# swyoon/Diffusion-by-MaxEntIRL

Hardware: AMD Instinct MI355X
Metric: images/sec (CIFAR-10 DDPM T=10 generation) (higher is better)
Workload: dtype bf16; 1 GPU; CIFAR-10 DDPM U-Net (35.7M params) VARSampler T=10 generation, 256 images/GPU/step, 3x32x32 (BASELINE configs[1]); noise drawn inside the step; global_batch=256, T=10, parallelism=dp1 (independent trajectories, no collective)

## Files before the change

diffusion-by-maxentirl_amd/dxmi_hip/_lib.py:

```python
import ctypes
import os

_HERE = os.path.dirname(os.path.abspath(__file__))
LIB_PATH = os.environ.get("DXMI_LIB") or os.path.join(_HERE, "libdxmi_hip.so")

c_void_p, c_int, c_float, c_int64 = ctypes.c_void_p, ctypes.c_int32, ctypes.c_float, ctypes.c_int64


class ConvDesc(ctypes.Structure):

    _fields_ = [
        ("in0", c_void_p), ("in1", c_void_p), ("wpacked", c_void_p), ("bias", c_void_p),
        ("addvec", c_void_p), ("residual", c_void_p), ("out", c_void_p),
        ("N", c_int), ("IH", c_int), ("IW", c_int), ("C0", c_int), ("C1", c_int),
        ("OH", c_int), ("OW", c_int), ("Cout", c_int),
        ("ksize", c_int), ("stride", c_int), ("pad", c_int), ("upsample", c_int), ("act", c_int),
        ("addvec_ld", c_int), ("in_mode", c_int), ("out_mode", c_int), ("variant", c_int),
        ("mask_src", c_void_p), ("mask_slope", c_float), ("gn_stats", c_void_p),
        ("gn_out", c_void_p), ("gn_gamma", c_void_p), ("gn_beta", c_void_p), ("gn_eps", c_float), ("gn_groups", c_int), ("gn_flags", c_int),
    ]


class PackItem(ctypes.Structure):

    _fields_ = [("w", c_void_p), ("dst", c_void_p), ("Cout", c_int), ("Cin", c_int), ("ksize", c_int), ("transpose_flip", c_int),
                ("k27", c_int)]


SIGNATURES = {
    "dxmi_last_error": (ctypes.c_char_p, []),
    "dxmi_version": (c_int, []),
    "dxmi_device_check": (c_int, []),
    "dxmi_set_tuning": (c_int, [ctypes.c_char_p, c_int]),
    "dxmi_get_tuning": (c_int, [ctypes.c_char_p, ctypes.POINTER(c_int)]),
    "dxmi_conv2d_fwd": (c_int, [ctypes.POINTER(ConvDesc), c_void_p]),
    "dxmi_conv2d_kernel_id": (c_int, [ctypes.POINTER(ConvDesc)]),
    "dxmi_conv2d_gn_stats_partials": (c_int, [ctypes.POINTER(ConvDesc)]),
    "dxmi_conv2d_gn_fuse_supported": (c_int, [ctypes.POINTER(ConvDesc)]),
    "dxmi_conv_ws_last_clock": (c_int, [ctypes.POINTER(ctypes.c_uint64)]),
    "dxmi_gn_block_stats_partials": (c_int, [c_int]),
    "dxmi_gn_block_stats": (c_int, [c_void_p, c_void_p, c_int, c_int, c_int, c_void_p]),
    "dxmi_gn_stats_fold": (c_int, [c_void_p, c_void_p, c_int, c_int, c_int, c_int, c_void_p]),
    "dxmi_groupnorm_apply": (c_int, [c_void_p, c_int, c_void_p, c_int, c_void_p, c_int, c_void_p, c_int, c_void_p, c_void_p, c_void_p, c_int,
                                     c_void_p, c_int, c_int, c_int, c_float, c_int, c_void_p]),
    "dxmi_groupnorm_apply_split": (c_int, [c_void_p, c_int, c_void_p, c_int, c_void_p, c_int, c_void_p, c_int, c_void_p, c_void_p, c_void_p, c_int,
                                           c_void_p, c_void_p, c_int, c_int, c_int, c_float, c_int, c_void_p]),
    "dxmi_groupnorm_silu_shortcut_supported": (c_int, [ctypes.POINTER(ConvDesc), c_int]),
    "dxmi_groupnorm_silu_shortcut": (c_int, [ctypes.POINTER(ConvDesc), c_void_p, c_int, c_void_p, c_int, c_void_p, c_void_p, c_int, c_float,
                                             c_int, c_void_p, c_void_p, c_void_p]),
    "dxmi_gn_blockstats_to_generic": (c_int, [c_void_p, c_int, c_int, c_void_p, c_int, c_int, c_void_p, c_int, c_int, c_int, c_void_p]),
    "dxmi_attention_fwd_lse_supported": (c_int, [c_int, c_int, c_int]),
    "dxmi_attention_fwd_lse": (c_int, [c_void_p, c_void_p, c_void_p, c_int, c_int, c_int, c_int, c_float, c_void_p]),
    "dxmi_attention_bwd_lse": (c_int, [c_void_p, c_void_p, c_void_p, c_void_p, c_void_p, c_void_p, c_int, c_int, c_int, c_int, c_float, c_void_p]),
    "dxmi_gn_ss_grads": (c_int, [c_void_p, c_void_p, c_int, c_void_p, c_void_p, c_void_p, c_void_p, c_void_p, c_int, c_int, c_void_p]),
    "dxmi_fid_stats_workspace_bytes": (c_int64, [c_int64, c_int]),
    "dxmi_fid_stats": (c_int, [c_void_p, c_int64, c_int, c_void_p, c_void_p, c_void_p, c_void_p]),
    "dxmi_knn_radii_workspace_bytes": (c_int64, [c_int64, c_int, c_int, c_int]),
    "dxmi_knn_radii": (c_int, [c_void_p, c_int64, c_int, c_int, c_int, c_void_p, c_void_p, c_void_p]),
    "dxmi_pr_membership_workspace_bytes": (c_int64, [c_int64, c_int64]),
    "dxmi_pr_membership": (c_int, [c_void_p, c_int64, c_void_p, c_void_p, c_int64, c_void_p, c_int, c_void_p, c_void_p, c_void_p, c_void_p]),
    "dxmi_inception_score_workspace_bytes": (c_int64, [c_int64, c_int, c_int]),
    "dxmi_inception_score": (c_int, [c_void_p, c_int64, c_int, c_void_p, c_int, c_int, c_void_p, c_void_p, c_void_p]),
    "dxmi_packed_conv_weight_bytes": (c_int64, [c_int, c_int, c_int, c_int]),
    "dxmi_pack_conv_weights": (c_int, [ctypes.POINTER(PackItem), c_int, c_void_p]),
    "dxmi_pack_conv_weight": (c_int, [c_void_p, c_void_p, c_int, c_int, c_int, c_int, c_int, c_void_p]),
    "dxmi_conv2d_wgrad_workspace_bytes": (c_int64, [c_int] * 6),
    "dxmi_conv2d_wgrad_plan": (c_int, [c_int] * 12 + [c_void_p]),
    "dxmi_conv2d_wgrad": (c_int, [c_void_p, c_int, c_void_p, c_int, c_void_p, c_void_p, c_void_p] + [c_int] * 11 + [c_void_p]),
    "dxmi_conv2d_wgrad_bias": (c_int, [c_void_p, c_int, c_void_p, c_int, c_void_p, c_void_p, c_void_p, c_void_p] + [c_int] * 11 + [c_void_p]),
    "dxmi_groupnorm_silu_bwd": (c_int, [c_void_p, c_int, c_void_p, c_int] + [c_void_p] * 9 + [c_int, c_int, c_int, c_float, c_int, c_void_p]),
    "dxmi_bgemm_bf16": (c_int, [c_void_p, c_void_p, c_void_p, c_int, c_int, c_int, c_int64, c_int64, c_int, c_int, c_int64, c_int64, c_int, c_int, c_int64, c_int64, c_int, c_int, c_float, c_int, c_int, c_void_p]),
    "dxmi_softmax_bwd": (c_int, [c_void_p, c_void_p, c_void_p, c_void_p, c_int64, c_int, c_void_p]),
    "dxmi_attention_bwd_supported": (c_int, [c_int, c_int, c_int]),
    "dxmi_attention_bwd_workspace_bytes": (c_int64, [c_int, c_int, c_int]),
    "dxmi_attention_bwd": (c_int, [c_void_p, c_void_p, c_void_p, c_void_p, c_void_p, c_int, c_int, c_int, c_int, c_float, c_void_p]),
    "dxmi_colsum_bf16": (c_int, [c_void_p, c_void_p, c_void_p, c_int64, c_int, c_int, c_void_p]),
    "dxmi_colsum_blocks_bf16": (c_int, [c_void_p, c_void_p, c_int64, c_int, c_int, c_void_p]),
    "dxmi_colsum_f32": (c_int, [c_void_p, c_void_p, c_int, c_int, c_int, c_void_p]),
    "dxmi_pool_act_bwd": (c_int, [c_void_p, c_void_p, c_void_p, c_int, c_int, c_int, c_int, c_int, c_float, c_void_p]),
    "dxmi_value_head_bwd": (c_int, [c_void_p, c_void_p, c_void_p, c_void_p, c_void_p, c_int, c_int, c_int, c_void_p]),
    "dxmi_groupnorm_silu_fwd": (c_int, [c_void_p, c_int, c_void_p, c_int, c_void_p, c_void_p, c_void_p,
                                        c_int, c_int, c_int, c_float, c_int, c_void_p]),
    "dxmi_attention_fwd": (c_int, [c_void_p, c_void_p, c_int, c_int, c_int, c_int, c_float, c_void_p]),
    "dxmi_attention_proj_supported": (c_int, [c_int, c_int, c_int]),
    "dxmi_pack_attn_proj_weight": (c_int, [c_void_p, c_void_p, c_void_p]),
    "dxmi_attention_proj_fwd": (c_int, [c_void_p, c_void_p, c_void_p, c_void_p, c_void_p, c_void_p, c_int, c_int, c_int, c_int, c_float, c_void_p]),
    "dxmi_attn_block_supported": (c_int, [c_int, c_int, c_int, c_int]),
    "dxmi_attn_block_packed_bytes": (c_int64, []),
    "dxmi_attn_block_pack": (c_int, [c_void_p] * 7 + [c_float, c_void_p, c_void_p]),
    "dxmi_attn_block_fwd": (c_int, [c_void_p, c_void_p, c_int, c_void_p, c_void_p, c_float, c_void_p, c_void_p, c_void_p, c_int, c_int, c_int, c_void_p]),
    "dxmi_timestep_embedding": (c_int, [c_void_p, c_void_p, c_int, c_int, c_int, c_float, c_void_p]),
    "dxmi_linear_fwd": (c_int, [c_void_p, c_void_p, c_void_p, c_void_p, c_int, c_int, c_int, c_int, c_int, c_void_p]),
    "dxmi_linear_splitk_slices": (c_int, [c_int, c_int, c_int]),
    "dxmi_linear_splitk": (c_int, [c_void_p, c_void_p, c_void_p, c_int, c_int, c_int, c_int, c_void_p]),
    "dxmi_var_step_fwd": (c_int, [c_void_p] * 10 + [c_int, c_int, c_int, c_void_p]),
    "dxmi_var_step_bwd": (c_int, [c_void_p] * 9 + [c_int, c_int, c_void_p]),
    "dxmi_edm_step_bwd": (c_int, [c_void_p] * 7 + [c_int, c_int, c_float, c_void_p]),
    "dxmi_var_gather_sched": (c_int, [c_void_p] * 9 + [c_int, c_int, c_void_p]),
    "dxmi_pool_act": (c_int, [c_void_p, c_void_p, c_int, c_int, c_int, c_int, c_int, c_int, c_void_p]),
    "dxmi_value_head": (c_int, [c_void_p, c_void_p, c_void_p, c_void_p, c_void_p, c_void_p, c_int, c_int, c_int, c_void_p]),
    "dxmi_groupnorm_silu_supported": (c_int, [c_int, c_int, c_int, c_int]),
    "dxmi_groupnorm_silu_bwd_supported": (c_int, [c_int, c_int, c_int, c_int]),
# ... 85 lines not shown
```

diffusion-by-maxentirl_amd/dxmi_hip/ops.py:

```python
import ctypes
import os

import torch

from . import _lib
from . import graph as _graph
from ._lib import ConvDesc, check, load

ACT_NONE, ACT_LEAKY02, ACT_RELU, ACT_SILU = 0, 1, 2, 3
IN_NHWC_BF16, IN_NCHW_F32_K27 = 0, 1
OUT_NHWC_BF16, OUT_NCHW_F32 = 0, 1


_RAW_STREAM = getattr(torch._C, "_cuda_getCurrentRawStream", None)
_GET_DEVICE = getattr(torch._C, "_cuda_getDevice", None)


def _stream():
    if _RAW_STREAM is not None and _GET_DEVICE is not None:
        return ctypes.c_void_p(_RAW_STREAM(_GET_DEVICE()))
    return ctypes.c_void_p(torch.cuda.current_stream().cuda_stream)


def _tree_fingerprint(module):
# ... 604 lines not shown
    while st.P > MAX_APPLY_PARTIALS:
        N, P, C2, _ = st.buf.shape
        PG = (P + group - 1) // group
        out = torch.empty((N, PG, C2, 2), dtype=torch.float32, device=st.buf.device)
        _prof("groupnorm", "fold", 0.0, 4.0 * (st.buf.numel() + out.numel()), lambda: check(
            load().dxmi_gn_stats_fold(_ptr(st.buf), _ptr(out), N, P, C2 * 2, group, _stream()), "dxmi_gn_stats_fold"))
        st = BlockStats(out, PG)
    return st


def block_stats(x):
    _need_cuda(x)
    N, H, W, C = x.shape
    assert x.dtype == torch.bfloat16 and x.is_contiguous()
    lib = load()
    P = int(lib.dxmi_gn_block_stats_partials(H * W))
    st = BlockStats(torch.empty((N, P, C // 2, 2), dtype=torch.float32, device=x.device), P)
    _prof("groupnorm", "block_stats", 0.0, 2.0 * x.numel(), lambda: check(
        lib.dxmi_gn_block_stats(_ptr(x), _ptr(st.buf), N, H * W, C, _stream()), "dxmi_gn_block_stats"))
    return fold_stats(st) if P > MAX_APPLY_PARTIALS else st


GN_APPLY_SPLIT = os.environ.get("DXMI_GN_APPLY_SPLIT", "0") == "1"


def groupnorm_apply(x, st, gamma, beta, *, in1=None, st1=None, groups=32, eps=1e-6, silu=True, out=None, scale_shift=None):
    _need_cuda(x, in1, gamma, beta, out, st.buf, st1.buf if st1 is not None else None, scale_shift)
    N, H, W, C0 = x.shape
    C1 = in1.shape[3] if in1 is not None else 0
    C = C0 + C1
    assert x.dtype == torch.bfloat16 and x.is_contiguous() and (in1 is None or (in1.is_contiguous() and st1 is not None))
    assert gamma.dtype == torch.float32 and beta.dtype == torch.float32 and gamma.numel() == C
    assert tuple(st.buf.shape) == (N, st.P, C0 // 2, 2) and (st1 is None or tuple(st1.buf.shape) == (N, st1.P, C1 // 2, 2))
    ss_ld = 0
    if scale_shift is not None:
        assert scale_shift.dtype == torch.float32 and scale_shift.stride(-1) == 1 and scale_shift.shape[1] == 2 * C
        ss_ld = scale_shift.stride(0)
    if out is None:
        out = torch.empty((N, H, W, C), dtype=torch.bfloat16, device=x.device)
    if GN_APPLY_SPLIT:
        ab = torch.empty((N, C, 2), dtype=torch.float32, device=x.device)
        _prof("groupnorm", "apply", 0.0, 4.0 * N * H * W * C, lambda: check(
            load().dxmi_groupnorm_apply_split(_ptr(x), C0, _ptr(st.buf), st.P, _ptr(in1), C1, _ptr(st1.buf) if st1 is not None else None,
                                              st1.P if st1 is not None else 0, _ptr(gamma), _ptr(beta), _ptr(scale_shift), ss_ld, _ptr(out),
                                              _ptr(ab), N, H * W, groups, float(eps), int(silu), _stream()), "dxmi_groupnorm_apply_split"))
        return out
    _prof("groupnorm", "apply", 0.0, 4.0 * N * H * W * C, lambda: check(
        load().dxmi_groupnorm_apply(_ptr(x), C0, _ptr(st.buf), st.P, _ptr(in1), C1, _ptr(st1.buf) if st1 is not None else None,
                                    st1.P if st1 is not None else 0, _ptr(gamma), _ptr(beta), _ptr(scale_shift), ss_ld, _ptr(out),
                                    N, H * W, groups, float(eps), int(silu), _stream()), "dxmi_groupnorm_apply"))
    return out


def groupnorm_silu(x, gamma, beta, *, in1=None, groups=32, eps=1e-6, silu=True, out=None, scale_shift=None, stats=None, saved=None):
    _need_cuda(x, in1, gamma, beta, out, scale_shift)
    N, H, W, C0 = x.shape
    C1 = in1.shape[3] if in1 is not None else 0
    if stats is not None and stats[0] is not None and (in1 is None or stats[1] is not None) \
            and ((C0 + C1) // groups) % 2 == 0 and C0 % 8 == 0 and C1 % 8 == 0:
        if saved is not None:
            saved.append(gn_blockstats_to_generic(stats[0], stats[1] if in1 is not None else None, N, H * W, C0, C1, groups))
        return groupnorm_apply(x, stats[0], gamma, beta, in1=in1, st1=stats[1] if in1 is not None else None, groups=groups,
                               eps=eps, silu=silu, out=out, scale_shift=scale_shift)
    if scale_shift is not None or not load().dxmi_groupnorm_silu_supported(C0, C1, H * W, groups):
        return groupnorm_generic(x, gamma, beta, in1=in1, groups=groups, eps=eps, silu=silu, out=out, scale_shift=scale_shift, saved=saved)
    assert x.dtype == torch.bfloat16 and x.is_contiguous()
    assert gamma.dtype == torch.float32 and beta.dtype == torch.float32 and gamma.numel() == C0 + C1
    if out is None:
        out = torch.empty((N, H, W, C0 + C1), dtype=torch.bfloat16, device=x.device)
    _prof("groupnorm", "resident", 0.0, 4.0 * N * H * W * (C0 + C1), lambda: check(
        load().dxmi_groupnorm_silu_fwd(_ptr(x), C0, _ptr(in1), C1, _ptr(gamma), _ptr(beta), _ptr(out), N, H * W,
                                       groups, float(eps), int(silu), _stream()), "dxmi_groupnorm_silu_fwd"))
    return out


def groupnorm_silu_shortcut(x, gamma, beta, pw, *, in1=None, bias=None, groups=32, eps=1e-6, silu=True, stats=None):
    _need_cuda(x, in1, gamma, beta, bias)
    if stats is None or stats[0] is None or (in1 is not None and stats[1] is None) or pw.k27 or pw.ksize != 1:
        return None
    N, H, W, C0 = x.shape
    C1 = in1.shape[3] if in1 is not None else 0
    C = C0 + C1
    if (C // groups) % 2 != 0 or C0 % 8 != 0 or C1 % 8 != 0:
        return None
    assert x.dtype == torch.bfloat16 and x.is_contiguous() and C == pw.Cin
    assert in1 is None or (in1.dtype == torch.bfloat16 and in1.is_contiguous() and in1.shape[:3] == x.shape[:3])
    assert gamma.dtype == torch.float32 and beta.dtype == torch.float32 and gamma.numel() == C and beta.numel() == C
    st0, st1 = stats[0], (stats[1] if in1 is not None else None)
    assert tuple(st0.buf.shape) == (N, st0.P, C0 // 2, 2) and (st1 is None or tuple(st1.buf.shape) == (N, st1.P, C1 // 2, 2))
    Cout = pw.Cout
    sc = torch.empty((N, H, W, Cout), dtype=torch.bfloat16, device=x.device)
    d = ConvDesc()
    d.in0, d.in1, d.wpacked = x.data_ptr(), (in1.data_ptr() if in1 is not None else None), pw.buf.data_ptr()
    d.bias = bias.data_ptr() if bias is not None else None
    d.out = sc.data_ptr()
    d.N, d.IH, d.IW, d.C0, d.C1, d.OH, d.OW, d.Cout = N, H, W, C0, C1, H, W, Cout
    d.ksize, d.stride, d.pad, d.upsample, d.act = 1, 1, 0, 0, ACT_NONE
    d.in_mode, d.out_mode = IN_NHWC_BF16, OUT_NHWC_BF16
    lib = load()
    key = ("gn_shortcut", N, H, W, C0, C1, Cout, groups, bias is not None)
    ok = _STATS_P.get(key)
    if ok is None:
        ok = _STATS_P[key] = int(lib.dxmi_groupnorm_silu_shortcut_supported(ctypes.byref(d), groups))
    if not ok:
        return None
    y = torch.empty((N, H, W, C), dtype=torch.bfloat16, device=x.device)
    ab = torch.empty((N, C, 2), dtype=torch.float32, device=x.device)
    px = N * H * W
    _prof("groupnorm", "gn_shortcut", 2.0 * px * C * Cout, 2.0 * (2 * px * C + px * Cout + C * Cout), lambda: check(
        lib.dxmi_groupnorm_silu_shortcut(ctypes.byref(d), _ptr(st0.buf), st0.P, _ptr(st1.buf) if st1 is not None else None,
                                         st1.P if st1 is not None else 0, _ptr(gamma), _ptr(beta), groups, float(eps), int(silu),
                                         _ptr(y), _ptr(ab), _stream()), "dxmi_groupnorm_silu_shortcut"))
    return y, sc


def gn_blockstats_to_generic(st0, st1, N, HW, C0, C1, groups=32):
    lib = load()
    ws = torch.empty(lib.dxmi_groupnorm_generic_workspace_bytes(N, HW, C0 + C1) // 4, dtype=torch.float32, device=st0.buf.device)
    check(lib.dxmi_gn_blockstats_to_generic(_ptr(st0.buf), st0.P, C0, _ptr(st1.buf) if st1 is not None else None, st1.P if st1 is not None else 0,
                                            C1, _ptr(ws), N, HW, groups, _stream()), "dxmi_gn_blockstats_to_generic")
    return ws


def groupnorm_generic(x, gamma, beta, *, in1=None, groups=32, eps=1e-5, silu=True, out=None, scale_shift=None, saved=None):
    _need_cuda(x, in1, gamma, beta, out, scale_shift)
    N, H, W, C0 = x.shape
    C1 = in1.shape[3] if in1 is not None else 0
    C = C0 + C1
    assert x.dtype == torch.bfloat16 and x.is_contiguous()
    if out is None:
        out = torch.empty((N, H, W, C), dtype=torch.bfloat16, device=x.device)
    ss_ld = 0
    if scale_shift is not None:
        assert scale_shift.dtype == torch.float32 and scale_shift.stride(-1) == 1 and scale_shift.shape[1] == 2 * C
        ss_ld = scale_shift.stride(0)
    lib = load()
    nbytes = lib.dxmi_groupnorm_generic_workspace_bytes(N, H * W, C)
    if saved is not None:
        ws = torch.empty(nbytes // 4, dtype=torch.float32, device=x.device)
        saved.append(ws)
    else:
        ws = _workspace(nbytes, x.device)
    _prof("groupnorm", "generic", 0.0, 4.0 * N * H * W * C, lambda: check(
        lib.dxmi_groupnorm_generic_fwd(_ptr(x), C0, _ptr(in1), C1, _ptr(gamma), _ptr(beta), _ptr(scale_shift), ss_ld, _ptr(out),
                                       _ptr(ws), N, H * W, groups, float(eps), int(silu), _stream()), "dxmi_groupnorm_generic_fwd"))
    return out


def groupnorm_generic_bwd(x, dy, gamma, beta, *, in1=None, add0=None, add1=None, groups=32, eps=1e-5, silu=True, scale_shift=None,
                          fwd_stats=None):
    _need_cuda(x, in1, dy, add0, add1, gamma, beta, scale_shift, fwd_stats)
    N, H, W, C0 = x.shape
    C1 = in1.shape[3] if in1 is not None else 0
    C = C0 + C1
    assert dy.dtype == torch.bfloat16 and dy.is_contiguous() and tuple(dy.shape) == (N, H, W, C)
    dx0 = torch.empty_like(x)
    dx1 = torch.empty_like(in1) if in1 is not None else None
    g = torch.empty((2, N, C), dtype=torch.float32, device=x.device)
    ss_ld = scale_shift.stride(0) if scale_shift is not None else 0
    lib = load()
    ws = _workspace(lib.dxmi_groupnorm_generic_bwd_workspace_bytes(N, H * W, C), x.device)
    if fwd_stats is not None:
        assert fwd_stats.dtype == torch.float32 and fwd_stats.numel() * 4 == lib.dxmi_groupnorm_generic_workspace_bytes(N, H * W, C)
    check(lib.dxmi_groupnorm_generic_bwd_saved(_ptr(x), C0, _ptr(in1), C1, _ptr(dy), _ptr(add0), _ptr(add1), _ptr(gamma), _ptr(beta),
                                               _ptr(scale_shift), ss_ld, _ptr(dx0), _ptr(dx1), _ptr(g), _ptr(fwd_stats), _ptr(ws), N, H * W,
                                               groups, float(eps), int(silu), _stream()), "dxmi_groupnorm_generic_bwd")
    if scale_shift is None:
        red = colsum_f32(g)
# ... 822 lines not shown
```

diffusion-by-maxentirl_amd/models/DxMI/unet_small.py:

```python
import os

import torch
import torch.nn as nn

from dxmi_hip import ops
from dxmi_hip._lib import DxmiError


def Normalize(in_channels):
    return nn.GroupNorm(num_groups=32, num_channels=in_channels, eps=1e-6, affine=True)


def _conv(cin, cout, k, stride=1, padding=0):
    return nn.Conv2d(cin, cout, kernel_size=k, stride=stride, padding=padding)


class Upsample(nn.Module):

    def __init__(self, in_channels, with_conv):
        super().__init__()
        self.with_conv = with_conv
        if with_conv:
            self.conv = _conv(in_channels, in_channels, 3, 1, 1)

# ... 144 lines not shown
                                         out=ops.pack_tensor(sum(b.out_channels for b in blocks), f32, dev))
            off = 0
            for b in blocks:
                pk[id(b), "toff"] = off
                off += b.out_channels
                pk[id(b), "conv1"] = ops.pack_conv_weight(b.conv1.weight)
                pk[id(b), "conv2"] = ops.pack_conv_weight(b.conv2.weight)
                if b.in_channels != b.out_channels:
                    sc = b.conv_shortcut if b.use_conv_shortcut else b.nin_shortcut
                    pk[id(b), "short"] = ops.pack_conv_weight(sc.weight)
            for m in self.modules():
                if isinstance(m, AttnBlock):
                    pk[id(m), "qkv"] = ops.pack_conv_weight(torch.cat([m.q.weight, m.k.weight, m.v.weight], 0))
                    pk[id(m), "qkv_bias"] = torch.cat([m.q.bias.detach(), m.k.bias.detach(), m.v.bias.detach()], 0,
                                                      out=ops.pack_tensor(3 * m.in_channels, f32, dev))
                    pk[id(m), "proj"] = ops.pack_conv_weight(m.proj_out.weight)
                    if m.in_channels == 256:
                        pk[id(m), "proj_attn"] = ops.pack_attn_proj_weight(m.proj_out.weight)
                        pk[id(m), "block"] = ops.attn_block_pack(m.q.weight, m.q.bias, m.k.weight, m.v.weight, m.v.bias,
                                                                 m.proj_out.weight, m.proj_out.bias, float(int(m.in_channels) ** (-0.5)))
                elif isinstance(m, (Upsample, Downsample)):
                    pk[id(m), "conv"] = ops.pack_conv_weight(m.conv.weight)
            pk["conv_in"] = ops.pack_conv_weight(self.conv_in.weight, k27=(self.in_channels == 3))
            pk["conv_out"] = ops.pack_conv_weight(self.conv_out.weight)
        assert dev.type == "cuda"
        self._pack_bufs = pb.buffers
        return pk

    @staticmethod
    def _same_storage(key, old_key):
        return old_key is not None and len(key) == len(old_key) and all(a[0] == b[0] for a, b in zip(key, old_key))

    def packed(self):
        key = self._param_key()
        if self._packed is None or key != self._packed_key:
            reuse = self._pack_bufs if (self._packed is not None and self._same_storage(key, self._packed_key)) else None
            self._packed, self._packed_key = self._pack(reuse=reuse), key
        return self._packed

    def refresh_packs(self):
        self.packed()
        if getattr(self, "_packed_t", None) is not None:
            from .unet_small_train import _pack_t
            _pack_t(self)

    def prepare_capture(self):
        if getattr(self, "_packed_t", None) is not None:
            for k in [k for k in self._packed_t if k not in self._packed_t_planned]:
                del self._packed_t[k]
        self.refresh_packs()

    FUSE_ATTN_PROJ = True
    FUSE_GN_SHORTCUT = os.environ.get("DXMI_GN_SHORTCUT", "1") != "0"
    FUSE_ATTN_BLOCK = True
    FUSE_GN_SMALL = True
    STREAM_GN_MIN_HW = 256

    def _conv_s(self, x, pw, **kw):
        out, st = ops.conv2d(x, pw, want_stats=True, **kw)
        if st is None and out.shape[1] * out.shape[2] >= self.STREAM_GN_MIN_HW:
            st = ops.block_stats(out)
        return out, st

    def _resblock(self, pk, b, x0, x1, tp, s0=None, s1=None, nxt=None):
        stream = x0.shape[1] * x0.shape[2] >= self.STREAM_GN_MIN_HW
        fused = None
        if isinstance(s0, _Normed):
            assert s0.norm is b.norm1 and x1 is None
            a0 = s0.y
        else:
            if self.FUSE_GN_SHORTCUT and stream and b.in_channels != b.out_channels and not b.use_conv_shortcut:
                fused = ops.groupnorm_silu_shortcut(x0, b.norm1.weight, b.norm1.bias, pk[id(b), "short"], in1=x1, bias=b.nin_shortcut.bias,
                                                    eps=1e-6, silu=True, stats=(s0, s1))
            if fused is not None:
                a0, sc = fused
            else:
                a0 = ops.groupnorm_silu(x0, b.norm1.weight, b.norm1.bias, in1=x1, eps=1e-6, silu=True, stats=(s0, s1))
        off = pk[id(b), "toff"]
        a = None
        if not stream and self.FUSE_GN_SMALL:
            h, a = ops.conv2d(a0, pk[id(b), "conv1"], bias=b.conv1.bias, addvec=tp[:, off:off + b.out_channels],
                              fuse_gn=(b.norm2.weight, b.norm2.bias, 32, 1e-6, True, False))
            sh = None
            if a is None and stream:
                sh = ops.block_stats(h)
        else:
            h, sh = ops.conv2d(a0, pk[id(b), "conv1"], bias=b.conv1.bias, addvec=tp[:, off:off + b.out_channels], want_stats=True)
        if a is None:
            a = ops.groupnorm_silu(h, b.norm2.weight, b.norm2.bias, eps=1e-6, silu=True, stats=(sh, None))
        if b.in_channels != b.out_channels:
            if fused is None:
                sc_mod = b.conv_shortcut if b.use_conv_shortcut else b.nin_shortcut
                sc = ops.conv2d(x0, pk[id(b), "short"], in1=x1, bias=sc_mod.bias)
        else:
            assert x1 is None
            sc = x0
        if stream:
            return self._conv_s(a, pk[id(b), "conv2"], bias=b.conv2.bias, residual=sc)
        if nxt is not None and self.FUSE_GN_SMALL:
            h, y = ops.conv2d(a, pk[id(b), "conv2"], bias=b.conv2.bias, residual=sc,
                              fuse_gn=(nxt[0].weight, nxt[0].bias, 32, 1e-6, nxt[1], True))
            return h, (None if y is None else _Normed(y, nxt[0]))
        return ops.conv2d(a, pk[id(b), "conv2"], bias=b.conv2.bias, residual=sc), None

    def _attn(self, pk, m, x, sx=None):
        N, H, W, C = x.shape
        if self.FUSE_ATTN_BLOCK and (id(m), "block") in pk and isinstance(sx, ops.BlockStats) and ops.attn_block_supported(H * W, C, 1):
            return ops.attn_block(x, sx, m.norm.weight, m.norm.bias, pk[id(m), "block"], eps=1e-6, want_stats=True)
        if isinstance(sx, _Normed):
            assert sx.norm is m.norm
            hn = sx.y
        else:
            hn = ops.groupnorm_silu(x, m.norm.weight, m.norm.bias, eps=1e-6, silu=False, stats=(sx, None))
        qkv = ops.conv2d(hn, pk[id(m), "qkv"], bias=pk[id(m), "qkv_bias"])
        if self.FUSE_ATTN_PROJ and (id(m), "proj_attn") in pk and ops.attention_proj_supported(H * W, C, 1):
            out, st = ops.attention_proj(qkv.view(N, H * W, 3 * C), pk[id(m), "proj_attn"], m.proj_out.bias, x, heads=1,
                                         scale=float(int(C) ** (-0.5)), want_stats=True)
            return out.view(N, H, W, C), (st if H * W >= self.STREAM_GN_MIN_HW else None)
        a = ops.attention(qkv.view(N, H * W, 3 * C), heads=1, scale=float(int(C) ** (-0.5)))
        if H * W >= self.STREAM_GN_MIN_HW:
            return self._conv_s(a.view(N, H, W, C), pk[id(m), "proj"], bias=m.proj_out.bias, residual=x)
        return ops.conv2d(a.view(N, H, W, C), pk[id(m), "proj"], bias=m.proj_out.bias, residual=x), None

    def forward(self, x, t, temb_rows=None):
        assert x.shape[2] == x.shape[3] == self.resolution
        if not x.is_cuda:
            raise DxmiError("models.DxMI.unet_small.Model runs only on the HIP device path (no CPU fallback)")
        if torch.is_grad_enabled() and (x.requires_grad or any(p.requires_grad for p in ops.fast_parameters(self))):
            from .unet_small_train import forward_with_grad
            return forward_with_grad(self, x, t)
# ... 76 lines not shown
```

include/dxmi_hip.h:

```cpp
#ifndef DXMI_HIP_H
#define DXMI_HIP_H

#include <stdint.h>

#ifdef __cplusplus
extern "C" {
#endif

#define DXMI_OK            0
#define DXMI_EINVAL       -1
#define DXMI_ELAUNCH      -2
#define DXMI_ENODEV       -3

#define DXMI_ACT_NONE      0
#define DXMI_ACT_LEAKY02   1
#define DXMI_ACT_RELU      2
#define DXMI_ACT_SILU      3

#define DXMI_IN_NHWC_BF16     0
#define DXMI_IN_NCHW_F32_K27  1
#define DXMI_IN_ROWS_F32      2
#define DXMI_OUT_NHWC_BF16    0
#define DXMI_OUT_NCHW_F32     1
#define DXMI_OUT_ROWS_F32     2
// ... 82 lines not shown
int dxmi_colsum_f32(const float* in, float* out, int32_t B, int32_t N, int32_t C, void* stream);

int dxmi_groupnorm_silu_bwd(const void* in0, int32_t C0, const void* in1, int32_t C1, const void* dy,
                            const void* add0, const void* add1, const float* gamma, const float* beta,
                            void* dx0, void* dx1, float* dgamma_part, float* dbeta_part, int32_t N,
                            int32_t HW, int32_t groups, float eps, int32_t apply_silu, void* stream);
int dxmi_groupnorm_silu_bwd_supported(int32_t C0, int32_t C1, int32_t HW, int32_t groups);

int dxmi_bgemm_bf16(const void* A, const void* B, void* C, int32_t M, int32_t N, int32_t K, int64_t a_b0,
                    int64_t a_b1, int32_t a_ld, int32_t a_kcontig, int64_t b_b0, int64_t b_b1, int32_t b_ld,
                    int32_t b_kcontig, int64_t c_b0, int64_t c_b1, int32_t c_ld, int32_t c_f32, float alpha,
                    int32_t outer, int32_t inner, void* stream);
int dxmi_softmax_bwd(const float* S, const float* dP, void* P, void* dS, int64_t rows, int32_t T,
                     void* stream);

int dxmi_attention_bwd_supported(int32_t T, int32_t C, int32_t heads);
int64_t dxmi_attention_bwd_workspace_bytes(int32_t N, int32_t T, int32_t heads);
int dxmi_attention_bwd(const void* qkv, const void* o, const void* dout, void* dqkv, void* workspace, int32_t N, int32_t T,
                       int32_t C, int32_t heads, float scale, void* stream);

int dxmi_attention_fwd_lse_supported(int32_t T, int32_t C, int32_t heads);
int dxmi_attention_fwd_lse(const void* qkv, void* out, float* lse, int32_t N, int32_t T, int32_t C, int32_t heads, float scale, void* stream);
int dxmi_attention_bwd_lse(const void* qkv, const void* o, const void* dout, void* dqkv, const float* lse_fwd, void* workspace, int32_t N,
                           int32_t T, int32_t C, int32_t heads, float scale, void* stream);

int dxmi_pool_act_bwd(const void* dout, const void* act_out, void* din, int32_t N, int32_t H, int32_t W,
                      int32_t C, int32_t pool, float slope, void* stream);
int dxmi_value_head_bwd(const void* feat, const float* w, const float* dy, void* dfeat, float* s,
                        int32_t N, int32_t HW, int32_t C, void* stream);

int dxmi_groupnorm_silu_fwd(const void* in0, int32_t C0, const void* in1, int32_t C1,
                            const float* gamma, const float* beta, void* out,
                            int32_t N, int32_t HW, int32_t groups, float eps,
                            int32_t apply_silu, void* stream);

int dxmi_gn_block_stats_partials(int32_t HW);
int dxmi_gn_block_stats(const void* x, float* stats, int32_t N, int32_t HW, int32_t C, void* stream);
int dxmi_gn_stats_fold(const float* stats, float* out, int32_t N, int32_t P, int32_t C, int32_t group, void* stream);
int dxmi_groupnorm_apply(const void* in0, int32_t C0, const float* stats0, int32_t P0, const void* in1, int32_t C1,
                         const float* stats1, int32_t P1, const float* gamma, const float* beta, const float* scale_shift,
                         int32_t ss_ld, void* out, int32_t N, int32_t HW, int32_t groups, float eps, int32_t apply_silu,
                         void* stream);

int dxmi_groupnorm_apply_split(const void* in0, int32_t C0, const float* stats0, int32_t P0, const void* in1, int32_t C1,
                               const float* stats1, int32_t P1, const float* gamma, const float* beta,
                               const float* scale_shift, int32_t ss_ld, void* out, float* ab_workspace, int32_t N, int32_t HW,
                               int32_t groups, float eps, int32_t apply_silu, void* stream);

int dxmi_groupnorm_silu_shortcut_supported(const dxmi_conv_desc* d, int32_t groups);
int dxmi_groupnorm_silu_shortcut(const dxmi_conv_desc* d, const float* stats0, int32_t P0, const float* stats1, int32_t P1,
                                 const float* gamma, const float* beta, int32_t groups, float eps, int32_t apply_silu, void* y,
                                 float* ab_workspace, void* stream);

int dxmi_gn_blockstats_to_generic(const float* stats0, int32_t P0, int32_t C0, const float* stats1, int32_t P1, int32_t C1,
                                  float* generic_stats, int32_t N, int32_t HW, int32_t groups, void* stream);

int dxmi_gn_ss_grads(const float* g, const float* scale_shift, int32_t ss_ld, const float* gamma, const float* beta,
                     float* d_scale_shift, float* dgamma, float* dbeta, int32_t N, int32_t C, void* stream);

int dxmi_attention_fwd(const void* qkv, void* out, int32_t N, int32_t T, int32_t C,
                       int32_t heads, float scale, void* stream);

int dxmi_attention_proj_supported(int32_t T, int32_t C, int32_t heads);
int dxmi_pack_attn_proj_weight(const float* w_oi, void* dst, void* stream);
int dxmi_attention_proj_fwd(const void* qkv, const void* wproj_packed, const float* bias, const void* residual, void* out,
                            float* gn_stats, int32_t N, int32_t T, int32_t C, int32_t heads, float scale, void* stream);

int dxmi_attn_block_supported(int32_t T, int32_t C, int32_t heads, int32_t groups);
int64_t dxmi_attn_block_packed_bytes(void);
int dxmi_attn_block_pack(const float* wq, const float* bq, const float* wk, const float* wv, const float* bv,
                         const float* wproj, const float* bproj, float scale, void* dst, void* stream);
int dxmi_attn_block_fwd(const void* x, const float* stats, int32_t P, const float* gamma, const float* beta, float eps,
                        const void* packed, void* out, float* out_stats, int32_t N, int32_t T, int32_t C, void* stream);

int dxmi_timestep_embedding(const float* t, float* out, int32_t N, int32_t dim, int32_t order,
                            float max_period, void* stream);
int dxmi_linear_fwd(const float* x, const void* wpacked, const float* bias, float* out,
                    int32_t P, int32_t K, int32_t M, int32_t pre_act, int32_t post_act,
                    void* stream);
int dxmi_linear_splitk_slices(int32_t P, int32_t K, int32_t M);
int dxmi_linear_splitk(const float* x, const void* wpacked, float* partials, int32_t P, int32_t K, int32_t M, int32_t pre_act,
                       void* stream);

int dxmi_var_step_fwd(const float* x, const float* eps, const float* z,
                      const float* xmul, const float* cmul, const float* sigma,
                      float* x_next, float* mean, float* control, float* logp,
                      int32_t N, int32_t CHW, int32_t assoc, void* stream);

int dxmi_var_step_bwd(const float* g_next, const float* g_mean, const float* g_control, const float* g_logp, const float* z,
                      const float* cmul, const float* sigma, float* d_eps, float* d_sigma, int32_t N, int32_t CHW, void* stream);

int dxmi_edm_step_bwd(const float* g_sample, const float* g_mean, const float* z, const float* sigma, const float* sigma_down,
                      float* d_model_out, float* d_sigma_up, int32_t N, int32_t CHW, float sigma_data, void* stream);

int dxmi_var_gather_sched(const int64_t* t, const float* continuous_steps,
                          const float* xmul_tab, const float* cmul_tab,
                          const float* log_betas_all, float* tau, float* xmul, float* cmul,
                          float* sigma, int32_t N, int32_t T, void* stream);

int dxmi_pool_act(const void* in, void* out, int32_t N, int32_t H, int32_t W, int32_t C,
                  int32_t pool, int32_t act, void* stream);
int dxmi_value_head(const void* in, const float* w, const float* b, const float* out_w,
                    const float* out_b, float* out, int32_t N, int32_t HW, int32_t C, void* stream);

int dxmi_groupnorm_silu_supported(int32_t C0, int32_t C1, int32_t HW, int32_t groups);
int64_t dxmi_groupnorm_generic_workspace_bytes(int32_t N, int32_t HW, int32_t C);
// ... 216 lines not shown
```

Before: 6761 images/s.

## Fuse GroupNorm stats, SiLU apply and 1x1 shortcut conv for small resolutions

Adds a single HIP kernel for the 4x4 and 8x8 resnet blocks with 512->256 channels. Each 64-pixel tile loads its input once, computes group statistics in-block, writes the normalized SiLU activation, and runs the 1x1 nin_shortcut GEMM with MFMA from LDS. This removes separate stats, apply and shortcut-conv launches and a re-read of the input on the small decoder levels. It is limited to one exact channel configuration and adds a large LDS footprint per block.

Result: no change. 6750 images/s (-0.2%).

```diff
diff --git a/diffusion-by-maxentirl_amd/csrc/gn_shortcut_small.hip b/diffusion-by-maxentirl_amd/csrc/gn_shortcut_small.hip
--- /dev/null
+++ b/diffusion-by-maxentirl_amd/csrc/gn_shortcut_small.hip
@@ -0,0 +1,256 @@
+#include "conv_common.h"
+#include <stdlib.h>
+
+namespace {
+
+constexpr int GSS_C = 512;
+constexpr int GSS_COUT = 256;
+constexpr int GSS_CPG = 16;
+constexpr int GSS_ROW = GSS_C * 2;
+constexpr int GSS_RAW = 64 * GSS_ROW;
+constexpr int GSS_RO = 4 * 64 * 128;
+constexpr int GSS_RED = 8 * 4 * 32 * 4;
+constexpr int GSS_STAT = 4 * 32 * 4;
+constexpr int GSS_LDS = GSS_RAW + GSS_RO + GSS_RED + GSS_STAT;
+constexpr int GSS_PF = 8;
+
+struct GssArgs {
+    const bf16* in0;
+    const bf16* in1;
+    const bf16* w;
+    const float* bias;
+    const float* gamma;
+    const float* beta;
+    bf16* y;
+    bf16* out;
+    int C0, C1;
+    long total_px;
+    float eps, inv_cnt;
+    int silu;
+};
+
+#define GSS_LO(w) __uint_as_float((w) << 16)
+#define GSS_HI(w) __uint_as_float((w) & 0xffff0000u)
+
+template <int IMGS>
+__global__ __launch_bounds__(256) void gn_shortcut_small_kernel(GssArgs p) {
+    constexpr int QI = 16 / IMGS;
+    extern __shared__ __attribute__((aligned(1024))) char smem[];
+    char* const raw = smem;
+    float* const red = reinterpret_cast<float*>(smem + GSS_RAW + GSS_RO);
+    float* const stat = reinterpret_cast<float*>(smem + GSS_RAW + GSS_RO + GSS_RED);
+
+    const int tid = threadIdx.x, lane = tid & 63, h = lane >> 5;
+    const int wave = __builtin_amdgcn_readfirstlane(tid >> 6);
+    char* const ro = smem + GSS_RAW + wave * (64 * 128);
+    const long P0 = (long)blockIdx.x * 64;
+
+    const int c = lane * 8;
+    const bool from0 = c < p.C0;
+    const bf16* const src = from0 ? p.in0 + c : p.in1 + (c - p.C0);
+    const int Cs = from0 ? p.C0 : p.C1;
+    u32x4 v[16];
+#pragma unroll
+    for (int q = 0; q < 16; ++q) {
+        const long gp = P0 + wave + 4 * q;
+        v[q] = u32x4{0u, 0u, 0u, 0u};
+        if (gp < p.total_px) v[q] = *reinterpret_cast<const u32x4*>(src + gp * Cs);
+    }
+    const bf16x8* const wf = reinterpret_cast<const bf16x8*>(p.w) + (size_t)(wave * 2) * 64 + lane;
+    constexpr int WSTEP = (GSS_COUT / 32) * 64;
+    bf16x8 a[GSS_PF][2];
+#pragma unroll
+    for (int ks = 0; ks < GSS_PF; ++ks) {
+        a[ks][0] = wf[(size_t)ks * WSTEP];
+        a[ks][1] = wf[(size_t)ks * WSTEP + 64];
+    }
+    float ga[8], be[8];
+    {
+        const f32x4 g0 = *reinterpret_cast<const f32x4*>(p.gamma + c), g1 = *reinterpret_cast<const f32x4*>(p.gamma + c + 4);
+        const f32x4 b0 = *reinterpret_cast<const f32x4*>(p.beta + c), b1 = *reinterpret_cast<const f32x4*>(p.beta + c + 4);
+#pragma unroll
+        for (int e = 0; e < 4; ++e) { ga[e] = g0[e]; ga[4 + e] = g1[e]; be[e] = b0[e]; be[4 + e] = b1[e]; }
+    }
+    f32x4 bv[2][4];
+#pragma unroll
+    for (int mb = 0; mb < 2; ++mb)
+#pragma unroll
+        for (int g = 0; g < 4; ++g) {
+            bv[mb][g] = f32x4{0.f, 0.f, 0.f, 0.f};
+            if (p.bias) bv[mb][g] = *reinterpret_cast<const f32x4*>(p.bias + wave * 64 + mb * 32 + 8 * g + 4 * h);
+        }
+
+#pragma unroll
+    for (int q = 0; q < 16; ++q) {
+        const int px = wave + 4 * q;
+        *reinterpret_cast<u32x4*>(raw + px * GSS_ROW + ((lane ^ (px & 15)) << 4)) = v[q];
+    }
+
+    const int gl = lane >> 1;
+    auto group_reduce = [&](float (&t)[IMGS][2]) {
+#pragma unroll
+        for (int i = 0; i < IMGS; ++i)
+#pragma unroll
+            for (int o = 0; o < 2; ++o) {
+                const float r = t[i][o] + __shfl_xor(t[i][o], 1, 64);
+                if ((lane & 1) == 0) red[((wave + 4 * o) * 4 + i) * 32 + gl] = r;
+            }
+        lds_barrier();
+        if (tid < IMGS * 32) {
+            const int i = tid >> 5, g = tid & 31;
+            float r = 0.f;
+#pragma unroll
+            for (int w = 0; w < 8; ++w) r += red[(w * 4 + i) * 32 + g];
+            stat[i * 32 + g] = r;
+        }
+        lds_barrier();
+#pragma unroll
+        for (int i = 0; i < IMGS; ++i) t[i][0] = stat[i * 32 + gl];
+    };
+    float mean[IMGS], rstd[IMGS], part[IMGS][2];
+#pragma unroll
+    for (int i = 0; i < IMGS; ++i)
+#pragma unroll
+        for (int o = 0; o < 2; ++o) {
+            float sum = 0.f;
+#pragma unroll
+            for (int q = i * QI + o; q < (i + 1) * QI; q += 2)
+#pragma unroll
+                for (int e = 0; e < 4; ++e) sum += GSS_LO(v[q][e]) + GSS_HI(v[q][e]);
+            part[i][o] = sum;
+        }
+    group_reduce(part);
+#pragma unroll
+    for (int i = 0; i < IMGS; ++i) {
+        mean[i] = part[i][0] * p.inv_cnt;
+#pragma unroll
+        for (int o = 0; o < 2; ++o) {
+            float ssq = 0.f;
+#pragma unroll
+            for (int q = i * QI + o; q < (i + 1) * QI; q += 2)
+#pragma unroll
+                for (int e = 0; e < 4; ++e) {
+                    const float d0 = GSS_LO(v[q][e]) - mean[i], d1 = GSS_HI(v[q][e]) - mean[i];
+                    ssq += d0 * d0 + d1 * d1;
+                }
+            part[i][o] = ssq;
+        }
+    }
+    group_reduce(part);
+#pragma unroll
+    for (int i = 0; i < IMGS; ++i) {
+        const float var = part[i][0] * p.inv_cnt;
+        rstd[i] = rsqrtf(var + p.eps);
+    }
+
+#pragma unroll
+    for (int i = 0; i < IMGS; ++i) {
+        float A[8], B[8];
+#pragma unroll
+        for (int e = 0; e < 8; ++e) {
+            A[e] = ga[e] * rstd[i];
+            B[e] = be[e] - mean[i] * A[e];
+        }
+#pragma unroll
+        for (int q = i * QI; q < (i + 1) * QI; ++q) {
+            const long gp = P0 + wave + 4 * q;
+            bf16x8 o;
+#pragma unroll
+            for (int e = 0; e < 4; ++e) {
+                float y0 = GSS_LO(v[q][e]) * A[2 * e] + B[2 * e];
+                float y1 = GSS_HI(v[q][e]) * A[2 * e + 1] + B[2 * e + 1];
+                if (p.silu) {
+                    y0 = dxmi_silu_fast(y0);
+                    y1 = dxmi_silu_fast(y1);
+                }
+                o[2 * e] = (bf16)y0;
+                o[2 * e + 1] = (bf16)y1;
+            }
+            if (gp < p.total_px) *reinterpret_cast<bf16x8*>(p.y + gp * GSS_C + c) = o;
+        }
+    }
+
+    f32x16 acc[2][2];
+#pragma unroll
+    for (int mb = 0; mb < 2; ++mb)
+#pragma unroll
+        for (int nb = 0; nb < 2; ++nb)
+#pragma unroll
+            for (int r = 0; r < 16; ++r) acc[mb][nb][r] = 0.f;
+    const char* const brow = raw + (lane & 31) * GSS_ROW;
+#pragma unroll
+    for (int ks = 0; ks < GSS_C / 16; ++ks) {
+        const int off = ((ks * 2 + h) ^ (lane & 15)) << 4;
+        const bf16x8 b0 = *reinterpret_cast<const bf16x8*>(brow + off);
+        const bf16x8 b1 = *reinterpret_cast<const bf16x8*>(brow + 32 * GSS_ROW + off);
+        const bf16x8 a0 = a[ks % GSS_PF][0], a1 = a[ks % GSS_PF][1];
+        if (ks + GSS_PF < GSS_C / 16) {
+            a[ks % GSS_PF][0] = wf[(size_t)(ks + GSS_PF) * WSTEP];
+            a[ks % GSS_PF][1] = wf[(size_t)(ks + GSS_PF) * WSTEP + 64];
+        }
+        acc[0][0] = __builtin_amdgcn_mfma_f32_32x32x16_bf16(a0, b0, acc[0][0], 0, 0, 0);
+        acc[0][1] = __builtin_amdgcn_mfma_f32_32x32x16_bf16(a0, b1, acc[0][1], 0, 0, 0);
+        acc[1][0] = __builtin_amdgcn_mfma_f32_32x32x16_bf16(a1, b0, acc[1][0], 0, 0, 0);
+        acc[1][1] = __builtin_amdgcn_mfma_f32_32x32x16_bf16(a1, b1, acc[1][1], 0, 0, 0);
+    }
+
+#pragma unroll
+    for (int nb = 0; nb < 2; ++nb) {
+        const int px = nb * 32 + (lane & 31);
+#pragma unroll
+        for (int mb = 0; mb < 2; ++mb)
+#pragma unroll
+            for (int g = 0; g < 4; ++g) {
+                bf16x4 o;
+#pragma unroll
+                for (int e = 0; e < 4; ++e) o[e] = (bf16)(acc[mb][nb][4 * g + e] + bv[mb][g][e]);
+                *reinterpret_cast<bf16x4*>(ro + px * 128 + (((mb * 4 + g) ^ ((px >> 1) & 7)) << 4) + 8 * h) = o;
+            }
+    }
+    asm volatile("s_waitcnt lgkmcnt(0)" ::: "memory");
+#pragma unroll
+    for (int i = 0; i < 8; ++i) {
+        const int px = i * 8 + (lane >> 3), s = lane & 7;
+        const bf16x8 o = *reinterpret_cast<const bf16x8*>(ro + px * 128 + ((s ^ ((px >> 1) & 7)) << 4));
+        const long gp = P0 + px;
+        if (gp < p.total_px) *reinterpret_cast<bf16x8*>(p.out + gp * GSS_COUT + wave * 64 + s * 8) = o;
+    }
+}
+
+bool gss_scope(const dxmi_conv_desc* d, int groups) {
+    if (!d || d->ksize != 1 || d->stride != 1 || d->pad != 0 || d->upsample || d->residual || d->addvec || d->mask_src || d->gn_stats ||
+        d->gn_out || d->act != DXMI_ACT_NONE || d->variant != 0 || d->in_mode != DXMI_IN_NHWC_BF16 || d->out_mode != DXMI_OUT_NHWC_BF16)
+        return false;
+    if (d->N <= 0 || d->IH != d->OH || d->IW != d->OW || d->OH != d->OW || (d->OH != 8 && d->OH != 4)) return false;
+    if (d->C0 <= 0 || d->C1 < 0 || d->C0 + d->C1 != GSS_C || d->C0 % 8 != 0 || d->Cout != GSS_COUT) return false;
+    return groups == GSS_C / GSS_CPG;
+}
+
+}
+
+extern "C" int dxmi_gn_shortcut_small_supported(const dxmi_conv_desc* d, int32_t groups) { return gss_scope(d, groups) ? 1 : 0; }
+
+extern "C" int dxmi_gn_shortcut_small(const dxmi_conv_desc* d, const float* gamma, const float* beta, int32_t groups, float eps,
+                                      int32_t apply_silu, void* y, void* stream) {
+    DXMI_CHECK_ARG(d && d->in0 && d->wpacked && d->out && y && gamma && beta, "dxmi_gn_shortcut_small: null pointer");
+    DXMI_CHECK_ARG(d->C1 <= 0 || d->in1, "dxmi_gn_shortcut_small: C1>0 needs in1");
+    if (!gss_scope(d, groups)) return 1;
+    const int HW = d->OH * d->OW;
+    GssArgs a;
+    a.in0 = (const bf16*)d->in0; a.in1 = (const bf16*)d->in1; a.w = (const bf16*)d->wpacked; a.bias = d->bias;
+    a.gamma = gamma; a.beta = beta; a.y = (bf16*)y; a.out = (bf16*)d->out;
+    a.C0 = d->C0; a.C1 = d->C1; a.total_px = (long)d->N * HW;
+    a.eps = eps; a.inv_cnt = 1.f / (float)(HW * GSS_CPG); a.silu = apply_silu ? 1 : 0;
+    const unsigned grid = (unsigned)((a.total_px + 63) / 64);
+    const hipStream_t st = (hipStream_t)stream;
+    static bool attr_set = false;
+    if (!attr_set) {
+        (void)hipFuncSetAttribute(reinterpret_cast<const void*>(gn_shortcut_small_kernel<1>), hipFuncAttributeMaxDynamicSharedMemorySize, GSS_LDS);
+        (void)hipFuncSetAttribute(reinterpret_cast<const void*>(gn_shortcut_small_kernel<4>), hipFuncAttributeMaxDynamicSharedMemorySize, GSS_LDS);
+        attr_set = true;
+    }
+    if (HW == 64) hipLaunchKernelGGL((gn_shortcut_small_kernel<1>), dim3(grid), dim3(256), GSS_LDS, st, a);
+    else hipLaunchKernelGGL((gn_shortcut_small_kernel<4>), dim3(grid), dim3(256), GSS_LDS, st, a);
+    DXMI_CHECK_LAUNCH("dxmi_gn_shortcut_small");
+    return DXMI_OK;
+}
diff --git a/diffusion-by-maxentirl_amd/dxmi_hip/_lib.py b/diffusion-by-maxentirl_amd/dxmi_hip/_lib.py
--- a/diffusion-by-maxentirl_amd/dxmi_hip/_lib.py
+++ b/diffusion-by-maxentirl_amd/dxmi_hip/_lib.py
@@ -48,6 +48,8 @@
     "dxmi_groupnorm_silu_shortcut_supported": (c_int, [ctypes.POINTER(ConvDesc), c_int]),
     "dxmi_groupnorm_silu_shortcut": (c_int, [ctypes.POINTER(ConvDesc), c_void_p, c_int, c_void_p, c_int, c_void_p, c_void_p, c_int, c_float,
                                              c_int, c_void_p, c_void_p, c_void_p]),
+    "dxmi_gn_shortcut_small_supported": (c_int, [ctypes.POINTER(ConvDesc), c_int]),
+    "dxmi_gn_shortcut_small": (c_int, [ctypes.POINTER(ConvDesc), c_void_p, c_void_p, c_int, c_float, c_int, c_void_p, c_void_p]),
     "dxmi_gn_blockstats_to_generic": (c_int, [c_void_p, c_int, c_int, c_void_p, c_int, c_int, c_void_p, c_int, c_int, c_int, c_void_p]),
     "dxmi_attention_fwd_lse_supported": (c_int, [c_int, c_int, c_int]),
     "dxmi_attention_fwd_lse": (c_int, [c_void_p, c_void_p, c_void_p, c_int, c_int, c_int, c_int, c_float, c_void_p]),
diff --git a/diffusion-by-maxentirl_amd/dxmi_hip/ops.py b/diffusion-by-maxentirl_amd/dxmi_hip/ops.py
--- a/diffusion-by-maxentirl_amd/dxmi_hip/ops.py
+++ b/diffusion-by-maxentirl_amd/dxmi_hip/ops.py
@@ -680,10 +680,16 @@
     return out
 
 
-def groupnorm_silu(x, gamma, beta, *, in1=None, groups=32, eps=1e-6, silu=True, out=None, scale_shift=None, stats=None, saved=None):
+def groupnorm_silu(x, gamma, beta, *, in1=None, groups=32, eps=1e-6, silu=True, out=None, scale_shift=None, stats=None, saved=None,
+                   shortcut=None):
     _need_cuda(x, in1, gamma, beta, out, scale_shift)
     N, H, W, C0 = x.shape
     C1 = in1.shape[3] if in1 is not None else 0
+    if shortcut is not None and out is None and scale_shift is None and saved is None and (stats is None or stats[0] is None):
+        r = _gn_shortcut_small(x, gamma, beta, shortcut[0], in1, shortcut[1], groups, eps, silu)
+        if r is not None:
+            shortcut[2].append(r[1])
+            return r[0]
     if stats is not None and stats[0] is not None and (in1 is None or stats[1] is not None) \
             and ((C0 + C1) // groups) % 2 == 0 and C0 % 8 == 0 and C1 % 8 == 0:
         if saved is not None:
@@ -704,7 +710,11 @@
 
 def groupnorm_silu_shortcut(x, gamma, beta, pw, *, in1=None, bias=None, groups=32, eps=1e-6, silu=True, stats=None):
     _need_cuda(x, in1, gamma, beta, bias)
-    if stats is None or stats[0] is None or (in1 is not None and stats[1] is None) or pw.k27 or pw.ksize != 1:
+    if pw.k27 or pw.ksize != 1:
+        return None
+    if stats is None or (stats[0] is None and stats[1] is None):
+        return _gn_shortcut_small(x, gamma, beta, pw, in1, bias, groups, eps, silu)
+    if stats[0] is None or (in1 is not None and stats[1] is None):
         return None
     N, H, W, C0 = x.shape
     C1 = in1.shape[3] if in1 is not None else 0
@@ -742,6 +752,40 @@
     return y, sc
 
 
+def _gn_shortcut_small(x, gamma, beta, pw, in1, bias, groups, eps, silu):
+    if pw.k27 or pw.ksize != 1 or x.dim() != 4:
+        return None
+    N, H, W, C0 = x.shape
+    C1 = in1.shape[3] if in1 is not None else 0
+    C, Cout = C0 + C1, pw.Cout
+    d = ConvDesc()
+    d.N, d.IH, d.IW, d.C0, d.C1, d.OH, d.OW, d.Cout = N, H, W, C0, C1, H, W, Cout
+    d.ksize, d.stride, d.pad, d.upsample, d.act = 1, 1, 0, 0, ACT_NONE
+    d.in_mode, d.out_mode = IN_NHWC_BF16, OUT_NHWC_BF16
+    d.in0 = d.wpacked = d.out = 16
+    lib = load()
+    key = ("gn_shortcut_small", H, W, C0, C1, Cout, groups)
+    ok = _STATS_P.get(key)
+    if ok is None:
+        ok = _STATS_P[key] = int(lib.dxmi_gn_shortcut_small_supported(ctypes.byref(d), groups))
+    if not ok:
+        return None
+    assert x.dtype == torch.bfloat16 and x.is_contiguous() and C == pw.Cin
+    assert in1 is None or (in1.dtype == torch.bfloat16 and in1.is_contiguous() and in1.shape[:3] == x.shape[:3])
+    assert gamma.dtype == torch.float32 and beta.dtype == torch.float32 and gamma.numel() == C and beta.numel() == C
+    assert bias is None or (bias.dtype == torch.float32 and bias.numel() == Cout)
+    y = torch.empty((N, H, W, C), dtype=torch.bfloat16, device=x.device)
+    sc = torch.empty((N, H, W, Cout), dtype=torch.bfloat16, device=x.device)
+    d.in0, d.in1, d.wpacked = x.data_ptr(), (in1.data_ptr() if in1 is not None else None), pw.buf.data_ptr()
+    d.bias = bias.data_ptr() if bias is not None else None
+    d.out = sc.data_ptr()
+    px = N * H * W
+    _prof("groupnorm", "gn_shortcut_small", 2.0 * px * C * Cout, 2.0 * (2 * px * C + px * Cout + C * Cout), lambda: check(
+        lib.dxmi_gn_shortcut_small(ctypes.byref(d), _ptr(gamma), _ptr(beta), groups, float(eps), int(silu), _ptr(y), _stream()),
+        "dxmi_gn_shortcut_small"))
+    return y, sc
+
+
 def gn_blockstats_to_generic(st0, st1, N, HW, C0, C1, groups=32):
     lib = load()
     ws = torch.empty(lib.dxmi_groupnorm_generic_workspace_bytes(N, HW, C0 + C1) // 4, dtype=torch.float32, device=st0.buf.device)
diff --git a/diffusion-by-maxentirl_amd/models/DxMI/unet_small.py b/diffusion-by-maxentirl_amd/models/DxMI/unet_small.py
--- a/diffusion-by-maxentirl_amd/models/DxMI/unet_small.py
+++ b/diffusion-by-maxentirl_amd/models/DxMI/unet_small.py
@@ -220,6 +220,7 @@
 
     FUSE_ATTN_PROJ = True
     FUSE_GN_SHORTCUT = os.environ.get("DXMI_GN_SHORTCUT", "1") != "0"
+    FUSE_GN_SHORTCUT_SMALL = os.environ.get("DXMI_GN_SHORTCUT_SMALL", "1") != "0"
     FUSE_ATTN_BLOCK = True
     FUSE_GN_SMALL = True
     STREAM_GN_MIN_HW = 256
@@ -243,7 +244,13 @@
             if fused is not None:
                 a0, sc = fused
             else:
-                a0 = ops.groupnorm_silu(x0, b.norm1.weight, b.norm1.bias, in1=x1, eps=1e-6, silu=True, stats=(s0, s1))
+                got = []
+                small = self.FUSE_GN_SHORTCUT_SMALL and not stream and b.in_channels != b.out_channels and not b.use_conv_shortcut
+                a0 = ops.groupnorm_silu(x0, b.norm1.weight, b.norm1.bias, in1=x1, eps=1e-6, silu=True, stats=(s0, s1),
+                                        shortcut=(pk[id(b), "short"], b.nin_shortcut.bias, got) if small else None)
+                if got:
+                    fused = (a0, got[0])
+                    sc = got[0]
         off = pk[id(b), "toff"]
         a = None
         if not stream and self.FUSE_GN_SMALL:
diff --git a/include/dxmi_hip.h b/include/dxmi_hip.h
--- a/include/dxmi_hip.h
+++ b/include/dxmi_hip.h
@@ -158,6 +158,10 @@
                                  const float* gamma, const float* beta, int32_t groups, float eps, int32_t apply_silu, void* y,
                                  float* ab_workspace, void* stream);
 
+int dxmi_gn_shortcut_small_supported(const dxmi_conv_desc* d, int32_t groups);
+int dxmi_gn_shortcut_small(const dxmi_conv_desc* d, const float* gamma, const float* beta, int32_t groups, float eps,
+                           int32_t apply_silu, void* y, void* stream);
+
 int dxmi_gn_blockstats_to_generic(const float* stats0, int32_t P0, int32_t C0, const float* stats1, int32_t P1, int32_t C1,
                                   float* generic_stats, int32_t N, int32_t HW, int32_t groups, void* stream);
 
```
